# exanauts/SqpSolver.jl

Hardware: AMD Instinct MI355X
Metric: QP subproblems/sec on batched ACOPF; fp64 KKT LDL^T TFLOPS vs MFMA peak (higher is better)
Workload: dtype f64

## Files before the change

include/sqphip_test_hooks.h:

```cpp
#ifndef SQPHIP_TEST_HOOKS_H
#define SQPHIP_TEST_HOOKS_H
#include "sqphip.h"
#ifdef __cplusplus
extern "C" {
#endif

int sqphip_mf_host_solve(int64_t n, int64_t m, int64_t nnzJ, const int64_t *jrow, const int64_t *jcol,
                         int64_t nnzH, const int64_t *hrow, const int64_t *hcol, const double *gL, const double *gU,
                         int32_t condense, const double *Jval, const double *Hval, const double *Dd,
                         const double *sigp, const double *hd, const int32_t *rtype, double hsc, double dw,
                         const double *rhs, double *sol, double *dinv_by_unknown, int32_t *npos);
double sqphip_mf_host_top2_err(void);
double sqphip_mf_host_spine_err(void);
int sqphip_mf_solve_test(sqphip_ctx *ctx, int32_t inst, const double *Jval, const double *Hval, const double *Dd,
                         const double *sigp, const double *hd, const int32_t *rtype, double hsc, double dw,
                         const double *rhs, double *sol_fused, double *sol_standalone, double *dinv_by_unknown);
int sqphip_mf_batch_test(sqphip_ctx *ctx, const int32_t *active, const double *Jval, const double *Hval, const double *Dd,
                         const double *sigp, const double *hd, const int32_t *rtype, const double *hsc, const double *dw,
                         const double *dw_last, const int32_t *fac_attempt, const double *rhs, double *sol_fused,
                         double *sol_standalone, double *dinv0, double *dinv1, int32_t *decision, double *dw_out);
int sqphip_mf_values_test(sqphip_ctx *ctx, const int32_t *active, const double *Jval, const double *Hval, const double *Dd,
                          const double *sigp, const double *hd, const int32_t *rtype, const double *hsc, const double *dw,
                          const double *dw_last, const int32_t *fac_attempt, double sentinel, double *vals0, double *vals1,
                          int64_t *nnzK);
int sqphip_mf_values_blocks(int64_t n, int64_t m, int64_t nnzJ, const int64_t *jrow, const int64_t *jcol, int64_t nnzH,
                            const int64_t *hrow, const int64_t *hcol, const double *gL, const double *gU, int32_t condense,
                            const double *Jval, const double *Hval, const double *Dd, const double *sigp, const double *hd,
                            const int32_t *rtype, double hsc, double dw, int32_t *blocks, int32_t cap_blocks,
                            int32_t *n_blocks, int32_t *item_ptr, int64_t cap_dest, int64_t *n_dest, int64_t *n_items,
                            double *vals_list, double *vals_block);
int sqphip_mf_census(const sqphip_ctx *ctx, int64_t *counts, char *names, int32_t cap, int32_t *n_kernels);
int sqphip_trans_inline_groups(const sqphip_ctx *ctx, int64_t *count);
int sqphip_mf_plan_info(int64_t n, int64_t m, int64_t nnzJ, const int64_t *jrow, const int64_t *jcol, int64_t nnzH,
                        const int64_t *hrow, const int64_t *hcol, const double *gL, const double *gU, int32_t condense,
                        int32_t batch, int32_t *fronts, int32_t cap_fronts, int32_t *n_fronts, int32_t *launches,
                        int32_t cap_launches, int32_t *n_launches, int64_t *top2_lds_bytes, int32_t *spine_fronts);
int sqphip_ldlt_factor_host(int32_t device, int32_t batch, int64_t N, double *A, double *dinv,
                            int32_t *npos);
int sqphip_ldlt_solve_host(int32_t device, int32_t batch, int64_t N, const double *A,
                           double *rhs);
int sqphip_ldlt_bench(int32_t device, int32_t batch, int64_t N, int32_t reps,
                      double *sec_per_factor, double *sec_trailing, int64_t *trailing_launches);
int sqphip_ldlt_tile_masks(int32_t batch, int64_t N, const double *A, int32_t Ts, uint8_t *tmask, int32_t *pair_ptr,
                           int32_t *pair_k, int32_t cap_k, int32_t *n_k);
int sqphip_ldlt_case_test(int32_t device, int32_t batch, int64_t N, const double *A, int32_t nan_upper, const double *rhs,
                          const int32_t *phase, int32_t want, int32_t Ts, int32_t no_tile_mask, double sentinel,
                          double *factor, double *dinv, int32_t *npos, double *b, double *v, double *x_fused,
                          double *x_standalone, int64_t *counts, char *names, int32_t cap, int64_t *info);

int sqphip_ldlt_stress(int32_t device, int32_t batch, int64_t N, int32_t reps, int32_t *mismatches);
int sqphip_mfma_f64_peak(int32_t device, double *tflops);

int sqphip_seat_peek(sqphip_ctx *ctx, int32_t inst, double *p, double *lambda, double *mult_x_U, double *mult_x_L,
                     double *slack, int32_t *moi_status);

#ifdef __cplusplus
}
#endif
#endif
// ... 1 lines not shown
```

sqpsolver.jl_amd/__init__.py:

```python
from . import acopf_synth
from . import dense_synth
from . import qcqp
from . import nlp_terms
from . import _lib
from . import host
from .host import (Context, QpData, QpHip, default_options, SqpHipError, kkt_order,
                   kkt_symbolic, mf_host_solve, mf_host_top2_err, mf_host_spine_err, mf_plan_info, mf_values_blocks)
```

sqpsolver.jl_amd/_lib.py:

```python
from __future__ import annotations

import ctypes as C
import os
import subprocess
import sys

_CSRC = os.path.join(os.path.dirname(os.path.abspath(__file__)), "csrc")
SO_PATH = os.path.join(_CSRC, "libsqphip.so")
if os.environ.get("SQPHIP_SO"):
    SO_PATH = os.path.abspath(os.environ["SQPHIP_SO"])
SOURCES = ["ldlt.hip", "kernel_api.hip", "ipm.hip", "acopf.hip", "sqp.hip", "api.hip", "order.hip", "symbolic.hip",
           "mfplan.hip", "mfront.hip", "comm.hip"]
HEADERS = ["sqphip_internal.hpp", "ctx.hpp", "sparse.hpp", "dev_util.hpp", "mf_dev.hpp", "sqp_dev.hpp", "acopf_dev.hpp", "qcqp_dev.hpp", "nlp_dev.hpp", os.path.join("..", "..", "include", "sqphip.h"),
           os.path.join("..", "..", "include", "sqphip_test_hooks.h")]

_lib = None


EXTRA_FLAGS = {"mfront.hip": ["-mllvm", "-amdgpu-mfma-vgpr-form", "-mllvm", "-pragma-unroll-threshold=131072"]}
_OBJ = os.path.join(_CSRC, "build")


def build(force: bool = False, verbose: bool = False) -> str:
    from concurrent.futures import ThreadPoolExecutor
# ... 166 lines not shown
            L.sqphip_acopf_set_dclines.argtypes = [vp, C.c_int32, dp]
            L.sqphip_kkt_order.argtypes = [C.c_int64, C.c_int64, C.c_int64, lp, lp, C.c_int64, lp, lp, dp, dp, C.c_int32,
                                           ip, ip, ip]
            L.sqphip_kkt_symbolic.argtypes = [C.c_int64, C.c_int64, C.c_int64, lp, lp, C.c_int64, lp, lp, dp, dp, C.c_int32,
                                              C.c_int32, C.c_int32, C.c_double, ip, C.POINTER(SymbolicStats)]
            L.sqphip_mf_host_solve.argtypes = [C.c_int64, C.c_int64, C.c_int64, lp, lp, C.c_int64, lp, lp, dp, dp, C.c_int32,
                                               dp, dp, dp, dp, dp, ip, C.c_double, C.c_double, dp, dp, dp, ip]
            L.sqphip_mf_host_top2_err.argtypes = []
            L.sqphip_mf_host_top2_err.restype = C.c_double
            L.sqphip_mf_host_spine_err.argtypes = []
            L.sqphip_mf_host_spine_err.restype = C.c_double
            L.sqphip_mf_solve_test.argtypes = [vp, C.c_int32, dp, dp, dp, dp, dp, ip, C.c_double, C.c_double, dp, dp, dp, dp]
            L.sqphip_mf_batch_test.argtypes = [vp, ip, dp, dp, dp, dp, dp, ip, dp, dp, dp, ip, dp, dp, dp, dp, dp, ip, dp]
            L.sqphip_mf_census.argtypes = [vp, lp, C.c_char_p, C.c_int32, ip]
            if not os.environ.get("SQPHIP_SO") or hasattr(L, "sqphip_mf_values_test"):
                L.sqphip_mf_values_test.argtypes = [vp, ip, dp, dp, dp, dp, dp, ip, dp, dp, dp, ip, C.c_double, dp, dp, lp]
                L.sqphip_mf_values_blocks.argtypes = [C.c_int64, C.c_int64, C.c_int64, lp, lp, C.c_int64, lp, lp, dp, dp, C.c_int32,
                                                      dp, dp, dp, dp, dp, ip, C.c_double, C.c_double, ip, C.c_int32, ip, ip,
                                                      C.c_int64, lp, lp, dp, dp]
            if hasattr(L, "sqphip_trans_inline_groups"):
                L.sqphip_trans_inline_groups.argtypes = [vp, lp]
            L.sqphip_mf_plan_info.argtypes = [C.c_int64, C.c_int64, C.c_int64, lp, lp, C.c_int64, lp, lp, dp, dp, C.c_int32,
                                              C.c_int32, ip, C.c_int32, ip, ip, C.c_int32, ip, lp, ip]
            L.sqphip_acopf_eval.argtypes = [vp, C.c_int32, dp, C.c_double, dp, dp, dp, dp, dp, dp]
            L.sqphip_sqp_reset.argtypes = [vp]
            L.sqphip_sqp_run.argtypes = [vp, C.c_int32]
            L.sqphip_sqp_get.argtypes = [vp, C.c_int32, dp, dp, dp, dp, dp, dp, ip, ip]
            L.sqphip_sqp_status.argtypes = [vp, ip, ip, ip]
            L.sqphip_sqp_trace.argtypes = [vp, C.c_int32, dp, C.c_int32, ip]
            L.sqphip_comm_unique_id.argtypes = [vp]
            L.sqphip_comm_init.argtypes = [vp, vp, C.c_int32, C.c_int32]
            L.sqphip_gather_status.argtypes = [vp, C.c_int32, ip, ip, ip]
            L.sqphip_comm_destroy.argtypes = [vp]
            L.sqphip_get_counters.argtypes = [vp, C.POINTER(Counters)]
            L.sqphip_get_mode_counters.argtypes = [vp, C.POINTER(C.c_int64)]
            L.sqphip_sqp_qp_log.argtypes = [vp, C.c_int32, ip, C.c_int32, ip]
            L.sqphip_sqp_last_request.argtypes = [vp, C.c_int32, ip, dp, dp, dp, dp, dp, dp, dp]
            L.sqphip_sqp_stream_begin.argtypes = [vp, C.c_int32]
            L.sqphip_sqp_stream_set.argtypes = [vp, C.c_int32] + [dp] * 8
            L.sqphip_sqp_stream_run.argtypes = [vp]
            L.sqphip_sqp_stream_get.argtypes = [vp, C.c_int32, dp, dp, ip, ip]
            L.sqphip_qcqp_stream_begin.argtypes = [vp, C.c_int32, C.c_int32]
            L.sqphip_qcqp_stream_set.argtypes = [vp, C.c_int32] + [dp] * 11
            L.sqphip_sqp_stream_get_full.argtypes = [vp, C.c_int32, dp, dp, dp, dp, dp, dp, ip, ip]
            if not os.environ.get("SQPHIP_SO") or hasattr(L, "sqphip_nlp_stream_begin"):
                L.sqphip_nlp_stream_begin.argtypes = [vp, C.c_int32, C.c_int32]
                L.sqphip_nlp_stream_set.argtypes = [vp, C.c_int32] + [dp] * 8
            L.sqphip_sqp_work.argtypes = [vp, C.POINTER(C.c_int64), C.POINTER(C.c_int64), C.POINTER(C.c_int64)]
            L.sqphip_reset_counters.argtypes = [vp]
            L.sqphip_set_timing.argtypes = [vp, C.c_int32]
            L.sqphip_get_kernel_times.argtypes = [vp, dp, C.POINTER(C.c_int64), C.c_int32]
        _lib = L
    return _lib


EXPORTS = [
    "sqphip_default_options", "sqphip_create", "sqphip_destroy", "sqphip_last_error",
    "sqphip_set_bounds", "sqphip_qp_solve", "sqphip_qp_stats",
    "sqphip_qp_solve_batch", "sqphip_qp_stats_batch", "sqphip_seat_peek", "sqphip_norm_violations_batch", "sqphip_kt_residuals_batch",
    "sqphip_norm_complementarity_batch", "sqphip_compute_phi_batch", "sqphip_compute_qmodel_batch",
    "sqphip_compute_derivative_full_batch", "sqphip_qp_termination", "sqphip_sqp_qp_log_term", "sqphip_get_termination_counters", "sqphip_norm_violations",
    "sqphip_kt_residuals", "sqphip_norm_complementarity", "sqphip_compute_phi",
    "sqphip_compute_qmodel", "sqphip_compute_derivative", "sqphip_compute_derivative_full", "sqphip_compute_mu_rule_dev",
    "sqphip_acopf_armijo", "sqphip_tr_update",
    "sqphip_kkt_order", "sqphip_kkt_symbolic", "sqphip_mf_host_solve", "sqphip_mf_host_top2_err", "sqphip_mf_host_spine_err", "sqphip_mf_solve_test", "sqphip_mf_batch_test", "sqphip_mf_values_test", "sqphip_mf_values_blocks", "sqphip_mf_census", "sqphip_trans_inline_groups", "sqphip_mf_plan_info", "sqphip_acopf_attach", "sqphip_acopf_attach_acr", "sqphip_acopf_attach_acwr", "sqphip_acopf_set_shunts", "sqphip_acopf_set_dclines", "sqphip_acopf_set_instance", "sqphip_dense_attach", "sqphip_dense_set_instance", "sqphip_qcqp_attach", "sqphip_qcqp_set_instance", "sqphip_nlp_attach", "sqphip_nlp_attach_affine", "sqphip_nlp_set_instance", "sqphip_acopf_eval", "sqphip_sqp_reset",
    "sqphip_sqp_run", "sqphip_sqp_get", "sqphip_sqp_status", "sqphip_sqp_trace",
    "sqphip_comm_available", "sqphip_comm_unique_id", "sqphip_comm_init", "sqphip_gather_status", "sqphip_comm_destroy",
    "sqphip_get_counters", "sqphip_get_mode_counters", "sqphip_sqp_work", "sqphip_sqp_stream_begin", "sqphip_sqp_stream_set", "sqphip_sqp_stream_run", "sqphip_sqp_stream_get", "sqphip_sqp_stream_assign", "sqphip_sqp_stream_append", "sqphip_sqp_stream_release", "sqphip_sqp_stream_run_some", "sqphip_qcqp_stream_begin", "sqphip_qcqp_stream_set", "sqphip_nlp_stream_begin", "sqphip_nlp_stream_set", "sqphip_sqp_stream_get_full", "sqphip_sqp_last_request", "sqphip_sqp_qp_log", "sqphip_reset_counters", "sqphip_set_timing", "sqphip_get_kernel_times", "sqphip_ldlt_factor_host",
    "sqphip_ldlt_solve_host", "sqphip_ldlt_bench", "sqphip_ldlt_stress", "sqphip_ldlt_tile_masks", "sqphip_ldlt_case_test", "sqphip_mfma_f64_peak", "sqphip_armijo_alpha", "sqphip_compute_mu_rule",
]
```

sqpsolver.jl_amd/csrc/api.hip:

```cpp
#include "ctx.hpp"
#include "qcqp_dev.hpp"
#include "nlp_dev.hpp"
#include <algorithm>
#include <array>
#include <chrono>
#include <cmath>
#include <cstring>
#include <tuple>
#include <unordered_map>

using namespace sqphip;

Ctx::~Ctx()
{
    lanes.clear();
    tm.flush();
    comm_release(*this);
    plan.destroy_lookahead();
    for (void *p : allocs) hipFree(p);
    if (h_counters) hipHostFree(h_counters);
    if (stg_h) hipHostFree(stg_h);
    if (side) { hipStreamDestroy(side); for (auto &e : evS) if (e) hipEventDestroy(e); for (auto &e : evC) if (e) hipEventDestroy(e); }
    if (stream && owns_stream) hipStreamDestroy(stream);
}
// ... 1858 lines not shown
        for (auto &s : S) { nqp += s.n_qp; nip += s.tot_ipm; nf += s.tot_fac; nsol += s.tot_sol; }
        c->n_qp = nqp; c->n_ipm_iter = nip; c->n_factor = nf;
        const double N = (double)C.d.Nf;
        c->kkt_order = C.d.Nf;
        c->lead_tiles = C.d.Ts;
        c->trailing_flops_per_factor = ldlt_trailing_flops(C.plan);
        c->ldlt_flops = (double)nf * N * N * N / 3.0;
        c->ldlt_seconds = C.tm.factor_seconds + lane_factor; c->trailing_seconds = C.tm.trailing_seconds + lane_trailing;
        c->solve_seconds = C.tm.solve_seconds + lane_solve; c->total_seconds = C.total_seconds;
        c->trailing_launches = C.tm.trailing_launches;
        c->n_sweeps = C.n_sweeps + lane_sweeps; c->n_solve = nsol; c->n_groups = C.lanes.empty() ? 1 : (int64_t)C.lanes.size();
        c->sparse = C.d.sparse; c->nnz_k = 0; c->nnz_l = 0; c->n_supernodes = 0; c->n_levels = 0; c->max_front = 0;
        c->factor_flops = 0; c->front_doubles = 0; c->cb_doubles = 0; c->factor_launches = 0; c->solve_launches = 0;
        c->nnz_l_top = 0; c->nnz_k_top = 0; c->cols_top = 0;
        if (C.d.sparse) {
            const SparseSym &Y = C.mfp().S;
            c->nnz_k = C.mfp().nnzK; c->nnz_l = Y.nnzL; c->n_supernodes = Y.ns; c->n_levels = Y.nlevels;
            c->max_front = Y.max_front; c->factor_flops = Y.flops; c->front_doubles = C.mfp().stride;
            long cb = 0;
            for (int q = 0; q < Y.ns; ++q) cb += (long)(Y.sn_nr[q] + 1) * Y.sn_nr[q] - (long)Y.sn_nr[q] * (Y.sn_nr[q] - 1) / 2;
            c->cb_doubles = cb;
            long lt = 0, kt = 0, nct = 0;
            for (int q = 0; q < Y.ns; ++q)
                if (Y.sn_level[q] >= C.mfp().narrow_level) {
                    const long nc = Y.sn_nc[q], nr = Y.sn_nr[q];
                    lt += nc * (nc - 1) / 2 + nc * nr; kt += C.mfp().asm_ptr[q + 1] - C.mfp().asm_ptr[q]; nct += nc;
                }
            c->nnz_l_top = lt; c->nnz_k_top = kt; c->cols_top = nct;
            c->factor_launches = (int64_t)(C.d.mf.sp_n > 0 ? C.mfp().fac_below + 1 : (int)C.mfp().fac.size());
            c->solve_launches = (int64_t)(C.mfp().fwd.size() + C.mfp().bwd.size() + (C.mfp().top.count > 0 ? 1 : 0));
            c->ldlt_flops = (double)nf * Y.flops;
        }
        return SQPHIP_OK;
    });
}

extern "C" int sqphip_get_mode_counters(sqphip_ctx *h, int64_t *out)
{
    if (!h || !out) return SQPHIP_EINVAL;
    return guarded(h, [&](Ctx &C) -> int {
        for (int k = 0; k < 12; ++k) out[k] = 0;
        if (!C.d.sst) return SQPHIP_OK;
        std::vector<SqpState> S((size_t)C.d.B);
        SQPHIP_HIP_OK(hipMemcpyAsync(S.data(), C.d.sst, sizeof(SqpState) * C.d.B, hipMemcpyDeviceToHost, C.stream));
        SQPHIP_HIP_OK(hipStreamSynchronize(C.stream));
        for (auto &s : S)
            for (int k = 0; k < 4; ++k) { out[3 * k] += s.md_qp[k]; out[3 * k + 1] += s.md_ipm[k]; out[3 * k + 2] += s.md_fac[k]; }
// ... 463 lines not shown
```

sqpsolver.jl_amd/csrc/mfplan.hip:

```cpp
#include "sparse.hpp"
#include "../../include/sqphip.h"
#include "../../include/sqphip_test_hooks.h"
#include <algorithm>
#include <cmath>
#include <cstdio>
#include <cstdlib>
#include <tuple>

namespace sqphip {

MfPlan mf_build_plan(int n, int m, const std::vector<int> &kpos, int mk, const std::vector<int> &hcolptr,
                     const std::vector<int> &hrowval, const std::vector<int> &jrowptr, const std::vector<int> &jrcol,
                     const std::vector<int> &jrslot, const SymOptions &opt)
{
    MfPlan P;
    std::vector<std::vector<int>> adj, before;
    kkt_graph(n, m, kpos, mk, hcolptr, hrowval, jrowptr, jrcol, adj, before);
    P.S = sparse_symbolic(n + mk, adj, before, opt);
    const SparseSym &S = P.S;
    P.off.resize(S.ns);
    for (int s = 0; s < S.ns; ++s) {
        const long fs = S.sn_nc[s] + S.sn_nr[s];
        P.off[s] = P.stride;
        P.stride += ((fs + 1) * fs + 1) / 2 * 2;
// ... 141 lines not shown
        }
        for (int s = 0; s < S.ns; ++s) P.ev_ptr[s + 1] += P.ev_ptr[s];
    }
    auto tiles = [&](int s) { return (S.sn_nc[s] + S.sn_nr[s] + 1 + 15) / 16; };
    auto cls = [&](int s) { const int T = tiles(s); return T <= 2 ? 1 : (T <= 6 ? T - 1 : (T <= 8 ? 7 : (T <= 13 ? 8 : 9))); };
    for (int l = 0; l < S.nlevels; ++l) {
        int cnt = 0, tmax = 0;
        for (int q = S.level_ptr[l]; q < S.level_ptr[l + 1]; ++q) { ++cnt; tmax = std::max(tmax, tiles(S.level_sn[q])); }
        const int merge_t = getenv("SQPHIP_MF_MERGE_T") ? atoi(getenv("SQPHIP_MF_MERGE_T")) : opt.merge_tiles;
        const bool merge = ((cnt <= 8 && tmax <= 8) || tmax <= merge_t) && !getenv("SQPHIP_MF_NO_LEVEL_MERGE");
        for (int c = 0; c < 10; ++c) {
            MfLaunch L{(int)P.sched.size(), 0, 0, 0, c, 0};
            L.level = l;
            for (int q = S.level_ptr[l]; q < S.level_ptr[l + 1]; ++q) {
                const int s = S.level_sn[q];
                if (merge ? c != tmax - 1 : cls(s) != c) continue;
                P.sched.push_back(s);
                L.count++;
                L.tiles = std::max(L.tiles, tiles(s));
            }
            if (!L.count) continue;
            if (!merge && c == 1) L.tiles = 2;
            if (!merge && c == 7) L.tiles = 8;
            P.fac.push_back(L);
        }
    }
    auto build_solve_launches = [&]() {
    P.sol_items.clear(); P.fwd.clear(); P.bwd.clear(); P.top = MfLaunch{0, 0, 256, 0, 0, 0};
    int top_maxfs = 64, top_lcap = 0;
    for (int l = 0; l < S.nlevels; ++l) {
        const bool top = l >= P.top_level;
        MfLaunch L{(int)P.sol_items.size() / 4, 0, 256, 0, 0, 0};
        int maxfs = 64, lcap = 0;
        std::vector<int> small;
        for (int q = S.level_ptr[l]; q < S.level_ptr[l + 1]; ++q) {
            const int s = S.level_sn[q], fs = S.sn_nc[s] + S.sn_nr[s];
            if (!big_solve) maxfs = std::max(maxfs, fs);
            if (fs > 64 && big_solve) {
                for (int t : {s, -2, -2, -2}) P.sol_items.push_back(t);
                maxfs = std::max(maxfs, fs);
                const int nc = S.sn_nc[s];
                if (nc <= 80) lcap = std::max(lcap, nc * nc);
            } else small.push_back(s);
        }
        for (size_t q = 0; q < small.size(); q += 4)
            for (size_t t = q; t < q + 4; ++t) P.sol_items.push_back(t < small.size() ? small[t] : -1);
// ... 135 lines not shown
                for (int t = 0; t < nr; ++t) P.sp_rel.push_back(S.rel[S.sn_rowptr[s] + t]);
                P.sp_rel.push_back(pfs);
                P.spine_stage = std::max(P.spine_stage, (nr + 1) * nr);
            }
            P.sp_fr.push_back(F);
        }
        if (ok && !P.sp_fr.empty()) {
            const int R = 16 * P.spine_T;
            P.spine_stage = (P.spine_stage + 1) / 2 * 2;
            P.spine_lds_bytes = 8L * ((long)R * R + 256 + 40 + R + 64 * 8 + P.spine_stage + 136);
            if (P.spine_lds_bytes > 160 * 1024 - 1024) ok = false;
        }
        if (!ok || P.sp_fr.empty()) { P.sp_fr.clear(); P.sp_ent.clear(); P.sp_src.clear(); P.sp_rel.clear(); P.spine_lds_bytes = 0; P.spine_level = S.nlevels; P.fac_below = (int)P.fac.size(); }
        if (getenv("SQPHIP_SYM_DUMP"))
            for (const MfSpineFront &F : P.sp_fr) {
                int hist[5] = {0, 0, 0, 0, 0};
                for (int t = F.ea_begin; t < F.ea_end; ++t) hist[std::min(4, P.sp_ent[t].src_end - P.sp_ent[t].src_begin)]++;
                fprintf(stderr, "  spine front %d: %d x %d, T %d, %d structural entries, %d receiving entries from the arena (1 / 2 / 3 / 4+ sources: %d / %d / %d / %d), handoff %d\n",
                        F.s, F.nc, F.nr, F.T, F.asm_end - F.asm_begin, F.ea_end - F.ea_begin, hist[1], hist[2], hist[3], hist[4], F.handoff);
            }
        if (getenv("SQPHIP_SYM_DUMP"))
            fprintf(stderr, "spine (factorisation): %d fronts from level %d, tallest %d tiles, %zu arena gather entries, LDS %ld bytes\n",
                    (int)P.sp_fr.size(), P.spine_level, P.spine_T, P.sp_ent.size(), P.spine_lds_bytes);
    }
    return P;
}

static inline double item_value(const MfItem &it, const MfValues &V)
{
    const double reg_p = 1e-8, reg_d = 1e-8;
    switch (it.type) {
    case MF_ITEM_H: return V.hsc * V.hv[it.a];
    case MF_ITEM_JKEPT: return V.rtype[it.row] != 0 ? V.jv[it.a] : 0.0;
    case MF_ITEM_PAIR: return V.rtype[it.row] != 0 ? V.jv[it.a] * V.jv[it.b] / (V.Dd[it.row] + reg_d) : 0.0;
    case MF_ITEM_VDIAG: return V.hd[it.a] + V.sigp[it.a] + V.dw + reg_p;
    default: return V.rtype[it.row] != 0 ? -(V.Dd[it.row] + reg_d) : -1.0;
    }
}

static double g_top2_err = -1.0;
static double g_spine_err = -1.0;

void mf_host_factor_solve(const MfPlan &P, const MfValues &V, const double *rhs, double *sol, double *dinv)
{
    const SparseSym &S = P.S;
    std::vector<double> F(P.stride, 0.0), x(S.nu), v(S.nu);
// ... 262 lines not shown
        (cap_launches > 0 && !launches))
        return SQPHIP_EINVAL;
    using namespace sqphip;
    const SymOptions so = mf_sym_options(batch);
    std::vector<double> jv, hv;
    const MfPlan P = host_plan(n, m, nnzJ, jrow, jcol, nnzH, hrow, hcol, gL, gU, condense, so, nullptr, nullptr, jv, hv);
    const SparseSym &S = P.S;
    std::vector<int> level(S.ns, 0);
    for (int l = 0; l < S.nlevels; ++l)
        for (int q = S.level_ptr[l]; q < S.level_ptr[l + 1]; ++q) level[S.level_sn[q]] = l;
    for (int f = 0; f < S.ns && f < cap_fronts; ++f) { fronts[3 * f] = S.sn_nc[f]; fronts[3 * f + 1] = S.sn_nr[f]; fronts[3 * f + 2] = level[f]; }
    for (int k = 0; k < (int)P.fac.size() && k < cap_launches; ++k) {
        const MfLaunch &L = P.fac[k];
        int tmin = 1 << 30;
        for (int q = L.begin; q < L.begin + L.count; ++q) tmin = std::min(tmin, (S.sn_nc[P.sched[q]] + S.sn_nr[P.sched[q]] + 1 + 15) / 16);
        launches[4 * k] = L.level; launches[4 * k + 1] = L.tiles; launches[4 * k + 2] = L.count; launches[4 * k + 3] = tmin;
    }
    if (n_fronts) *n_fronts = S.ns;
    if (n_launches) *n_launches = (int32_t)P.fac.size();
    if (top2_lds_bytes) *top2_lds_bytes = P.top2_lds_bytes;
    if (spine_fronts) *spine_fronts = (int32_t)P.sp_fr.size();
    return SQPHIP_OK;
}
```

sqpsolver.jl_amd/csrc/mfront.hip:

```cpp
#include "ctx.hpp"
#include "dev_util.hpp"
#include "mf_dev.hpp"
#include <cstdlib>
#include <mutex>

namespace sqphip {

#ifdef SQPHIP_MF_TRACE
__device__ long long g_mf_trace[1 << 16][8];
#define MF_TR(i) if (inst == 0 && threadIdx.x == 0 && s < (1 << 16)) g_mf_trace[s][i] = (long long)wall_clock64();
__device__ long long g_mf_trace2[1 << 12][16];
#define MF_TRW(i) if (W == 0 && trs >= 0 && trs < (1 << 12) && lane == 0) g_mf_trace2[trs][i] = (long long)clock64();
__device__ long long g_mf_trace3[1 << 12][16];
#define MF_TRS(i) if (inst == 0 && tid == 0 && s < (1 << 12)) g_mf_trace3[s][i] = (long long)clock64();
#define MF_TR2S(a, b) if (inst == 0 && lane == 0 && j < 64 && wave < 2) g_mf_trace3[(do_fwd ? 64 : 0) + j][wave == 0 ? (a) : (b)] = (long long)clock64();
#define MF_TR2W(c) if (trj >= 0 && lane == 0) g_mf_trace3[trj][c] = (long long)clock64();
#define MF_TRSP(c) if (inst == 0 && cand == 0 && tid == 0 && k < 64) g_mf_trace3[128 + k][c] = (long long)wall_clock64();
#else
#define MF_TR(i)
#define MF_TRW(i)
#define MF_TRS(i)
#define MF_TR2S(a, b)
#define MF_TR2W(c)
#define MF_TRSP(c)
// ... 1753 lines not shown
    big(reinterpret_cast<const void *>(k_mf_front<6, 4, true>)); big(reinterpret_cast<const void *>(k_mf_front<7, 4, true>));
    big(reinterpret_cast<const void *>(k_mf_front<8, 4, true>)); big(reinterpret_cast<const void *>(k_mf_front<6, 8, true>));
    big(reinterpret_cast<const void *>(k_mf_front<7, 8, true>)); big(reinterpret_cast<const void *>(k_mf_front<8, 8, true>));
    big(reinterpret_cast<const void *>(k_mf_fwd2<true>)); big(reinterpret_cast<const void *>(k_mf_bwd2<true>));
    big(reinterpret_cast<const void *>(k_mf_fwd2<false>)); big(reinterpret_cast<const void *>(k_mf_bwd2<false>));
    big(reinterpret_cast<const void *>(k_mf_solve_top2));
    big(reinterpret_cast<const void *>(k_mf_spine));
    (void)hipGetLastError();
    C.mf_big_lds = ok;
}

void mf_values(Ctx &C, int want)
{
    const DV &d = C.d;
    hipStream_t s = C.stream;
    const int nb = d.mf.fronts1 && d.spec_mode != 0 ? 2 * d.B : d.B;
    const bool serial = d.mf.nvblk == 0 || (getenv("SQPHIP_MF_VALUES_SERIAL") && atoi(getenv("SQPHIP_MF_VALUES_SERIAL")) != 0);
    C.tm.open(s); C.mf_census[MFK_VALUES]++;
    if (serial) hipLaunchKernelGGL(k_mf_values_serial, dim3((d.mf.nnzK + 255) / 256, nb), dim3(256), 0, s, d, want);
    else hipLaunchKernelGGL(k_mf_values, dim3(d.mf.nvblk, nb), dim3(MF_VBLK_ITEMS), 0, s, d, want);
    C.tm.close(KC_VALUES, s);
}

void mf_factor(Ctx &C, int want, bool with_rhs, bool values_done)
{
    const DV &d = C.d;
    hipStream_t s = C.stream;
    static const bool v1 = getenv("SQPHIP_MF_V1") != nullptr;
    const int wr = (int)with_rhs;
    const int nb = d.mf.fronts1 && d.spec_mode != 0 ? 2 * d.B : d.B;
    if (!v1 && !values_done) mf_values(C, want);
    const bool stat = !(getenv("SQPHIP_MF_STATIC") && atoi(getenv("SQPHIP_MF_STATIC")) == 0);
    const bool packed = !(getenv("SQPHIP_MF_F2_PACKED") && atoi(getenv("SQPHIP_MF_F2_PACKED")) == 0);
    const bool spine = !v1 && d.mf.sp_n > 0 && C.mf_big_lds;
    int li = 0, cls_open = -1;
    for (const MfLaunch &L : C.mfp().fac) {
        if (spine && li++ >= C.mfp().fac_below) break;
        const int cls = L.level >= C.mfp().narrow_level ? KC_FRONTS_TOP : KC_FRONTS_LOW;
        if (cls != cls_open) { if (cls_open >= 0) C.tm.close(cls_open, s); C.tm.open(s); cls_open = cls; }
        const dim3 grid(L.count, nb);
        const int T = L.tiles;
        if (v1 || T > 13) { C.mf_census[MFK_FACTOR_R1]++; hipLaunchKernelGGL((k_mf_factor<256, true>), grid, dim3(256), 0, s, d, L.begin, want, wr); continue; }
#define MF_GENERIC(NW, MAXT, IMG) do { constexpr int kid_ = mf_factor2_kid(NW, MAXT, IMG); static_assert(kid_ >= 0, "census: no counter"); C.mf_census[kid_]++; \
        if (IMG && packed) hipLaunchKernelGGL((k_mf_factor2<NW, MAXT, IMG, IMG>), grid, dim3(64 * NW), 8 * mf_factor2_lds_doubles(T, IMG, true), s, d, L.begin, want, wr, T); \
        else hipLaunchKernelGGL((k_mf_factor2<NW, MAXT, IMG, false>), grid, dim3(64 * NW), 8 * mf_factor2_lds_doubles(T, IMG, false), s, d, L.begin, want, wr, T); } while (0)
#define MF_STATIC(TT, NW, IMG) do { constexpr int kid_ = mf_front_kid(TT, NW, IMG); static_assert(kid_ >= 0, "census: no counter"); C.mf_census[kid_]++; hipLaunchKernelGGL((k_mf_front<TT, NW, IMG>), grid, dim3(64 * NW), 8 * (size_t)mf_front_lds_doubles(TT, NW, IMG), s, d, L.begin, want, wr); } while (0)
        const int stat_min = getenv("SQPHIP_MF_STATIC_MIN") ? atoi(getenv("SQPHIP_MF_STATIC_MIN")) : (L.count <= 8 && L.level >= C.mfp().narrow_level ? 1 : 4);
        const bool nw8 = !(getenv("SQPHIP_MF_NW8") && atoi(getenv("SQPHIP_MF_NW8")) == 0);
        const int nw4 = L.count <= 8 ? (getenv("SQPHIP_MF_NW4") ? atoi(getenv("SQPHIP_MF_NW4")) : 3) : 0;
        const bool big_img = C.mf_big_lds && !(getenv("SQPHIP_MF_BIG_LDSIMG") && atoi(getenv("SQPHIP_MF_BIG_LDSIMG")) == 0);
        static const int stat_max = getenv("SQPHIP_MF_STATIC_MAX") ? atoi(getenv("SQPHIP_MF_STATIC_MAX")) : 12;
        if (!stat || T > stat_max || T > 12 || T < stat_min) {
            if (T <= 2) MF_GENERIC(1, 3, true);
            else if (T <= 4) MF_GENERIC(2, 5, true);
            else if (T <= 5) MF_GENERIC(4, 4, true);
            else if (T <= 8) MF_GENERIC(4, 9, false);
            else MF_GENERIC(8, 12, false);
            continue;
        }
        switch (T) {
        case 1: MF_STATIC(1, 1, true); break;
        case 2: MF_STATIC(2, 1, true); break;
        case 3: MF_STATIC(3, 1, true); break;
        case 4: if (nw4 & 1) MF_STATIC(4, 4, true); else MF_STATIC(4, 2, true); break;
        case 5: if (nw4 & 2) MF_STATIC(5, 4, true); else MF_STATIC(5, 2, true); break;
        case 6: if (big_img && L.count <= 8) { if (nw8) MF_STATIC(6, 8, true); else MF_STATIC(6, 4, true); } else MF_STATIC(6, 4, false); break;
        case 7: if (big_img && L.count <= 8) { if (nw8) MF_STATIC(7, 8, true); else MF_STATIC(7, 4, true); } else MF_STATIC(7, 4, false); break;
        case 8: if (big_img && L.count <= 8) { if (nw8) MF_STATIC(8, 8, true); else MF_STATIC(8, 4, true); } else MF_STATIC(8, 4, false); break;
        case 9: MF_STATIC(9, 8, false); break;
        case 10: MF_STATIC(10, 8, false); break;
        case 11: MF_STATIC(11, 8, false); break;
        default: MF_STATIC(12, 8, false); break;
        }
#undef MF_GENERIC
#undef MF_STATIC
    }
    if (cls_open >= 0) C.tm.close(cls_open, s);
    if (spine) { C.tm.open(s); C.mf_census[MFK_SPINE]++; hipLaunchKernelGGL(k_mf_spine, dim3(1, nb), dim3(MF_SP_NT), (size_t)C.mfp().spine_lds_bytes, s, d, want, wr); C.tm.close(KC_FRONTS_TOP, s); }
    C.mf_factor_launches += spine ? (long)C.mfp().fac_below + 1 : (long)C.mfp().fac.size();
}

bool mf_solve_tests_inertia(const Ctx &C)
{
    static const bool off = getenv("SQPHIP_MF_INERTIA_KERNEL") != nullptr;
    return !off && C.d.sparse && C.d.mf.top_n > 0 && !mf_generic_solves() && !(C.d.B >= (getenv("SQPHIP_MF_INST_SOLVE_MIN") ? atoi(getenv("SQPHIP_MF_INST_SOLVE_MIN")) : (1 << 30)));
}

void mf_solve(Ctx &C, int want, bool skip_fwd, bool inertia, int also)
{
    const DV &d = C.d;
    hipStream_t s = C.stream;
// ... 49 lines not shown
```

sqpsolver.jl_amd/csrc/sparse.hpp:

```cpp
#pragma once
#include <cstdint>
#include <cstdlib>
#include <vector>

namespace sqphip {

struct SparseSym {
    int nu = 0;
    std::vector<int> pos, inv;
    int ns = 0;
    std::vector<int> sn_first, sn_nc, sn_nr, sn_rowptr, sn_rows, sn_parent, sn_level;
    std::vector<int> col2sn;
    std::vector<int> rel;
    std::vector<int> child_ptr, child;
    std::vector<long> front_off;
    long front_total = 0;
    int nlevels = 0;
    std::vector<int> level_ptr, level_sn;
    long nnzL = 0;
    long nnzL_exact = 0;
    double flops = 0;
    double flops_exact = 0;
    int max_front = 0, max_nc = 0;
};
// ... 19 lines not shown
    return so;
}

SparseSym sparse_symbolic(int nu, const std::vector<std::vector<int>> &adj, const std::vector<std::vector<int>> &before,
                          const SymOptions &opt);

void kkt_graph(int n, int m, const std::vector<int> &kpos, int mk, const std::vector<int> &hcolptr,
               const std::vector<int> &hrowval, const std::vector<int> &jrowptr, const std::vector<int> &jrcol,
               std::vector<std::vector<int>> &adj, std::vector<std::vector<int>> &before);

enum { MF_ITEM_H = 0,
       MF_ITEM_JKEPT = 1,
       MF_ITEM_PAIR = 2,
       MF_ITEM_VDIAG = 3,
       MF_ITEM_RDIAG = 4 };
struct MfItem { int type, row, a, b; };

constexpr int MF_VBLK_ITEMS = 256;
struct MfValBlock { int dest0, item0, ndest, nitems; };

struct MfFrontDesc { int nc, nr, first, rowptr, off, asm_begin, asm_end, ea_begin, ea_end, ev_begin, ev_end, pad; };
struct MfGather { int where, src_begin, src_end, src0; };

struct MfLaunch { int begin, count, threads, lds_bytes, cls, tiles; int wimg = -1, lds2 = 0, hasbig = 1; int level = 0; };

struct MfTopFront { int s, nc, nr, first, off, ll, xloc, uoff, gptr, gsrc0, nsrc, rloc, lbuf, pad0, pad1, pad2; };

struct MfSpineFront { int s, nc, nr, first, off, T, asm_begin, asm_end, ea_begin, ea_end, handoff, rel, pad0, pad1, pad2, pad3; };

struct MfPlan {
    SparseSym S;
    std::vector<long> off;
    long stride = 0;
    std::vector<int> asm_ptr, dest_loc, item_ptr;
    std::vector<MfItem> items;
    std::vector<MfItem> vitems;
    std::vector<MfValBlock> vblk;
    std::vector<int> dest_rc;
    std::vector<int> ea_ptr, ea_rc, ea_src_ptr, ea_src;
    std::vector<int> ev_ptr, ev_idx, ev_src_ptr, ev_src;
    std::vector<int> sol_items;
    std::vector<MfFrontDesc> desc;
    std::vector<MfGather> ea_ent, ev_ent;
    std::vector<int> sched;
    std::vector<MfLaunch> fac, fwd, bwd;
    MfLaunch top{0, 0, 256, 0, 0, 0};
    int top_level = 0;
    std::vector<MfTopFront> top_fr;
    std::vector<int> top_gptr, top_gsrc, top_rows, top_ext;
    int top_xtotal = 0, top_utotal = 0, top_buf0 = 0, top_buf1 = 0;
    long top2_lds_bytes = 0;
    long nnzK = 0;
    int spine_level = 0, spine_T = 0;
    int narrow_level = 0;
    std::vector<MfSpineFront> sp_fr;
    std::vector<MfGather> sp_ent;
    std::vector<int> sp_src, sp_rel;
    long spine_lds_bytes = 0;
    int spine_stage = 0;
    int fac_below = 0;
};

MfPlan mf_build_plan(int n, int m, const std::vector<int> &kpos, int mk, const std::vector<int> &hcolptr,
                     const std::vector<int> &hrowval, const std::vector<int> &jrowptr, const std::vector<int> &jrcol,
                     const std::vector<int> &jrslot, const SymOptions &opt);

struct MfValues { const double *hv, *jv, *Dd, *sigp, *hd; const int *rtype; double hsc, dw; };
void mf_host_factor_solve(const MfPlan &P, const MfValues &V, const double *rhs, double *sol, double *dinv);
// ... 3 lines not shown
```

sqpsolver.jl_amd/host.py:

```python
from __future__ import annotations

import ctypes as C
import dataclasses
import math
import numpy as np

from . import _lib

MODE_QP, MODE_FR, MODE_SOC, MODE_LP, MODE_L1QP, MODE_INFEAS = range(6)
LOCALLY_SOLVED, LOCALLY_INFEASIBLE, ITERATION_LIMIT, NUMERICAL_ERROR = 4, 5, 11, 20
_OK = (1, 7, 10, 4)
_INFEAS = (2, 5)

_dp = C.POINTER(C.c_double)


def _d(a):
    return None if a is None else a.ctypes.data_as(_dp)


def _f(a):
    return None if a is None else np.ascontiguousarray(a, dtype=np.float64)


# ... 57 lines not shown
        raise SqpHipError(f"sqphip_mf_host_solve failed ({rc})")
    return sol, dinv, npos.value


def mf_host_top2_err() -> float:
    return float(_lib.lib().sqphip_mf_host_top2_err())


def mf_host_spine_err() -> float:
    return float(_lib.lib().sqphip_mf_host_spine_err())


def mf_plan_info(n, m, jrow, jcol, hrow, hcol, gL, gU, condense=1, batch=1):
    L = _lib.lib()
    jr, jc, hr, hc = (np.ascontiguousarray(a, dtype=np.int64) for a in (jrow, jcol, hrow, hcol))
    nf, nl, top, sp = C.c_int32(), C.c_int32(), C.c_int64(), C.c_int32()
    args = (n, m, len(jr), _l(jr), _l(jc), len(hr), _l(hr), _l(hc), _d(_f(gL)), _d(_f(gU)), int(condense), int(batch))
    if L.sqphip_mf_plan_info(*args, None, 0, C.byref(nf), None, 0, C.byref(nl), C.byref(top), C.byref(sp)) != 0:
        raise SqpHipError("sqphip_mf_plan_info failed")
    fr = np.zeros((nf.value, 3), dtype=np.int32); la = np.zeros((nl.value, 4), dtype=np.int32)
    if L.sqphip_mf_plan_info(*args, _i(fr), nf.value, C.byref(nf), _i(la), nl.value, C.byref(nl), C.byref(top), C.byref(sp)) != 0:
        raise SqpHipError("sqphip_mf_plan_info failed")
    return fr, la, top.value, sp.value


def mf_values_blocks(n, m, jrow, jcol, hrow, hcol, gL, gU, condense=1, values=None):
    L = _lib.lib()
    jr, jc, hr, hc = (np.ascontiguousarray(a, dtype=np.int64) for a in (jrow, jcol, hrow, hcol))
    nb, nd, ni = C.c_int32(), C.c_int64(), C.c_int64()
    head = (n, m, len(jr), _l(jr), _l(jc), len(hr), _l(hr), _l(hc), _d(_f(gL)), _d(_f(gU)), int(condense))
    none = (None, None, None, None, None, None, 0.0, 0.0)
    if L.sqphip_mf_values_blocks(*head, *none, None, 0, C.byref(nb), None, 0, C.byref(nd), C.byref(ni), None, None) != 0:
        raise SqpHipError("sqphip_mf_values_blocks failed")
    blocks = np.zeros((nb.value, 4), dtype=np.int32); ptr = np.zeros(nd.value + 1, dtype=np.int32)
    out = {"blocks": blocks, "item_ptr": ptr, "n_items": ni.value, "vals_list": None, "vals_block": None}
    vals = none; vl = vb = None
    if values is not None:
        jval, hval, Dd, sigp, hd, rtype, hsc, dw = values
        rt = np.ascontiguousarray(rtype, dtype=np.int32)
        vals = (_d(_f(jval)), _d(_f(hval)), _d(_f(Dd)), _d(_f(sigp)), _d(_f(hd)), _i(rt), float(hsc), float(dw))
        vl = np.zeros(nd.value); vb = np.zeros(nd.value)
    if L.sqphip_mf_values_blocks(*head, *vals, _i(blocks) if nb.value else None, nb.value, C.byref(nb), _i(ptr), nd.value,
                                 C.byref(nd), C.byref(ni), _d(vl) if vl is not None else None,
                                 _d(vb) if vb is not None else None) != 0:
        raise SqpHipError("sqphip_mf_values_blocks failed")
    if values is not None:
# ... 593 lines not shown
```

Baseline: 10160.

## Defer multifrontal factor fronts into later compatible launches to cut launch count

Adds a planning pass that moves every front of a factor launch into later launches with the same kernel selection, provided each is still below its parent's level. A launch whose fronts can all be moved is removed, so fewer level-by-level factor kernels run and the remaining ones get wider grids. The pass is on by default, can be switched with an environment variable, and runs only when there is no spine. It records each launch's small/narrow properties so kernel choice stays the same after the merge. It also adds a test hook that reports the front-to-launch mapping, and the cost accounting now uses the launch's level instead of the front's own level.

```diff
diff --git a/include/sqphip_test_hooks.h b/include/sqphip_test_hooks.h
--- a/include/sqphip_test_hooks.h
+++ b/include/sqphip_test_hooks.h
@@ -35,6 +35,9 @@
                         const int64_t *hrow, const int64_t *hcol, const double *gL, const double *gU, int32_t condense,
                         int32_t batch, int32_t *fronts, int32_t cap_fronts, int32_t *n_fronts, int32_t *launches,
                         int32_t cap_launches, int32_t *n_launches, int64_t *top2_lds_bytes, int32_t *spine_fronts);
+int sqphip_mf_front_launches(int64_t n, int64_t m, int64_t nnzJ, const int64_t *jrow, const int64_t *jcol, int64_t nnzH,
+                             const int64_t *hrow, const int64_t *hcol, const double *gL, const double *gU, int32_t condense,
+                             int32_t batch, int32_t *fronts, int32_t cap_fronts, int32_t *n_fronts);
 int sqphip_ldlt_factor_host(int32_t device, int32_t batch, int64_t N, double *A, double *dinv,
                             int32_t *npos);
 int sqphip_ldlt_solve_host(int32_t device, int32_t batch, int64_t N, const double *A,
diff --git a/sqpsolver.jl_amd/__init__.py b/sqpsolver.jl_amd/__init__.py
--- a/sqpsolver.jl_amd/__init__.py
+++ b/sqpsolver.jl_amd/__init__.py
@@ -5,4 +5,4 @@
 from . import _lib
 from . import host
 from .host import (Context, QpData, QpHip, default_options, SqpHipError, kkt_order,
-                   kkt_symbolic, mf_host_solve, mf_host_top2_err, mf_host_spine_err, mf_plan_info, mf_values_blocks)
+                   kkt_symbolic, mf_host_solve, mf_host_top2_err, mf_host_spine_err, mf_plan_info, mf_front_launches, mf_values_blocks)
diff --git a/sqpsolver.jl_amd/_lib.py b/sqpsolver.jl_amd/_lib.py
--- a/sqpsolver.jl_amd/_lib.py
+++ b/sqpsolver.jl_amd/_lib.py
@@ -212,6 +212,9 @@
                 L.sqphip_trans_inline_groups.argtypes = [vp, lp]
             L.sqphip_mf_plan_info.argtypes = [C.c_int64, C.c_int64, C.c_int64, lp, lp, C.c_int64, lp, lp, dp, dp, C.c_int32,
                                               C.c_int32, ip, C.c_int32, ip, ip, C.c_int32, ip, lp, ip]
+            if not os.environ.get("SQPHIP_SO") or hasattr(L, "sqphip_mf_front_launches"):
+                L.sqphip_mf_front_launches.argtypes = [C.c_int64, C.c_int64, C.c_int64, lp, lp, C.c_int64, lp, lp, dp, dp, C.c_int32,
+                                                       C.c_int32, ip, C.c_int32, ip]
             L.sqphip_acopf_eval.argtypes = [vp, C.c_int32, dp, C.c_double, dp, dp, dp, dp, dp, dp]
             L.sqphip_sqp_reset.argtypes = [vp]
             L.sqphip_sqp_run.argtypes = [vp, C.c_int32]
@@ -253,7 +256,7 @@
     "sqphip_kt_residuals", "sqphip_norm_complementarity", "sqphip_compute_phi",
     "sqphip_compute_qmodel", "sqphip_compute_derivative", "sqphip_compute_derivative_full", "sqphip_compute_mu_rule_dev",
     "sqphip_acopf_armijo", "sqphip_tr_update",
-    "sqphip_kkt_order", "sqphip_kkt_symbolic", "sqphip_mf_host_solve", "sqphip_mf_host_top2_err", "sqphip_mf_host_spine_err", "sqphip_mf_solve_test", "sqphip_mf_batch_test", "sqphip_mf_values_test", "sqphip_mf_values_blocks", "sqphip_mf_census", "sqphip_trans_inline_groups", "sqphip_mf_plan_info", "sqphip_acopf_attach", "sqphip_acopf_attach_acr", "sqphip_acopf_attach_acwr", "sqphip_acopf_set_shunts", "sqphip_acopf_set_dclines", "sqphip_acopf_set_instance", "sqphip_dense_attach", "sqphip_dense_set_instance", "sqphip_qcqp_attach", "sqphip_qcqp_set_instance", "sqphip_nlp_attach", "sqphip_nlp_attach_affine", "sqphip_nlp_set_instance", "sqphip_acopf_eval", "sqphip_sqp_reset",
+    "sqphip_kkt_order", "sqphip_kkt_symbolic", "sqphip_mf_host_solve", "sqphip_mf_host_top2_err", "sqphip_mf_host_spine_err", "sqphip_mf_solve_test", "sqphip_mf_batch_test", "sqphip_mf_values_test", "sqphip_mf_values_blocks", "sqphip_mf_census", "sqphip_trans_inline_groups", "sqphip_mf_plan_info", "sqphip_mf_front_launches", "sqphip_acopf_attach", "sqphip_acopf_attach_acr", "sqphip_acopf_attach_acwr", "sqphip_acopf_set_shunts", "sqphip_acopf_set_dclines", "sqphip_acopf_set_instance", "sqphip_dense_attach", "sqphip_dense_set_instance", "sqphip_qcqp_attach", "sqphip_qcqp_set_instance", "sqphip_nlp_attach", "sqphip_nlp_attach_affine", "sqphip_nlp_set_instance", "sqphip_acopf_eval", "sqphip_sqp_reset",
     "sqphip_sqp_run", "sqphip_sqp_get", "sqphip_sqp_status", "sqphip_sqp_trace",
     "sqphip_comm_available", "sqphip_comm_unique_id", "sqphip_comm_init", "sqphip_gather_status", "sqphip_comm_destroy",
     "sqphip_get_counters", "sqphip_get_mode_counters", "sqphip_sqp_work", "sqphip_sqp_stream_begin", "sqphip_sqp_stream_set", "sqphip_sqp_stream_run", "sqphip_sqp_stream_get", "sqphip_sqp_stream_assign", "sqphip_sqp_stream_append", "sqphip_sqp_stream_release", "sqphip_sqp_stream_run_some", "sqphip_qcqp_stream_begin", "sqphip_qcqp_stream_set", "sqphip_nlp_stream_begin", "sqphip_nlp_stream_set", "sqphip_sqp_stream_get_full", "sqphip_sqp_last_request", "sqphip_sqp_qp_log", "sqphip_reset_counters", "sqphip_set_timing", "sqphip_get_kernel_times", "sqphip_ldlt_factor_host",
diff --git a/sqpsolver.jl_amd/csrc/api.hip b/sqpsolver.jl_amd/csrc/api.hip
--- a/sqpsolver.jl_amd/csrc/api.hip
+++ b/sqpsolver.jl_amd/csrc/api.hip
@@ -1904,7 +1904,7 @@
             c->cb_doubles = cb;
             long lt = 0, kt = 0, nct = 0;
             for (int q = 0; q < Y.ns; ++q)
-                if (Y.sn_level[q] >= C.mfp().narrow_level) {
+                if (C.mfp().fac[C.mfp().launch_of[q]].level >= C.mfp().narrow_level) {
                     const long nc = Y.sn_nc[q], nr = Y.sn_nr[q];
                     lt += nc * (nc - 1) / 2 + nc * nr; kt += C.mfp().asm_ptr[q + 1] - C.mfp().asm_ptr[q]; nct += nc;
                 }
diff --git a/sqpsolver.jl_amd/csrc/mfplan.hip b/sqpsolver.jl_amd/csrc/mfplan.hip
--- a/sqpsolver.jl_amd/csrc/mfplan.hip
+++ b/sqpsolver.jl_amd/csrc/mfplan.hip
@@ -187,6 +187,7 @@
             if (!L.count) continue;
             if (!merge && c == 1) L.tiles = 2;
             if (!merge && c == 7) L.tiles = 8;
+            L.small = L.count <= 8;
             P.fac.push_back(L);
         }
     }
@@ -368,6 +369,66 @@
         if (getenv("SQPHIP_SYM_DUMP"))
             fprintf(stderr, "spine (factorisation): %d fronts from level %d, tallest %d tiles, %zu arena gather entries, LDS %ld bytes\n",
                     (int)P.sp_fr.size(), P.spine_level, P.spine_T, P.sp_ent.size(), P.spine_lds_bytes);
+    }
+    {
+        const int defer = getenv("SQPHIP_MF_DEFER") ? atoi(getenv("SQPHIP_MF_DEFER")) : 1;
+        const int nl = (int)P.fac.size();
+        std::vector<std::vector<int>> mem(nl);
+        P.launch_of0.assign(S.ns, -1);
+        for (int k = 0; k < nl; ++k)
+            for (int q = P.fac[k].begin; q < P.fac[k].begin + P.fac[k].count; ++q) { mem[k].push_back(P.sched[q]); P.launch_of0[P.sched[q]] = k; }
+        std::vector<char> alive(nl, 1);
+        if (defer != 0 && P.sp_fr.empty()) {
+            std::vector<int> width(nl, 0);
+            for (int k = 0; k < nl; ++k) {
+                int fs = -1;
+                for (int s : mem[k]) {
+                    const int h = S.sn_nc[s] + S.sn_nr[s];
+                    if (h > fs || (h == fs && S.sn_nc[s] > width[k])) { fs = h; width[k] = S.sn_nc[s]; }
+                }
+            }
+            std::vector<int> dest;
+            for (int a = 0; a < nl; ++a) {
+                const MfLaunch &A = P.fac[a];
+                dest.clear();
+                for (int s : mem[a]) {
+                    const int p = S.sn_parent[s], bound = p >= 0 ? S.sn_level[p] : S.nlevels;
+                    int best = -1;
+                    for (int b = a + 1; b < nl && P.fac[b].level < bound; ++b) {
+                        const MfLaunch &B = P.fac[b];
+                        if (!alive[b] || B.level <= A.level || !mf_same_selection(A, B, P.narrow_level)) continue;
+                        if (best < 0 || defer != 2 || width[b] >= width[best]) best = b;
+                    }
+                    if (best < 0) break;
+                    dest.push_back(best);
+                }
+                if (dest.size() != mem[a].size()) continue;
+                for (size_t t = 0; t < dest.size(); ++t) mem[dest[t]].push_back(mem[a][t]);
+                mem[a].clear(); alive[a] = 0;
+            }
+            std::vector<MfLaunch> fac;
+            P.sched.clear();
+            for (int k = 0; k < nl; ++k) {
+                if (!alive[k]) continue;
+                MfLaunch L = P.fac[k];
+                L.begin = (int)P.sched.size(); L.count = (int)mem[k].size();
+                P.sched.insert(P.sched.end(), mem[k].begin(), mem[k].end());
+                fac.push_back(L);
+            }
+            P.fac.swap(fac);
+            P.fac_below = (int)P.fac.size();
+        }
+        P.launch_of.assign(S.ns, -1);
+        for (int k = 0; k < (int)P.fac.size(); ++k)
+            for (int q = P.fac[k].begin; q < P.fac[k].begin + P.fac[k].count; ++q) P.launch_of[P.sched[q]] = k;
+        if (getenv("SQPHIP_SYM_DUMP")) {
+            for (int s = 0; s < S.ns; ++s)
+                if (alive[P.launch_of0[s]] == 0)
+                    fprintf(stderr, "  deferred: front %d (%d x %d, level %d, parent's level %d) from launch %d to launch %d (level %d)\n", s, S.sn_nc[s],
+                            S.sn_nr[s], S.sn_level[s], S.sn_parent[s] >= 0 ? S.sn_level[S.sn_parent[s]] : -1, P.launch_of0[s], P.launch_of[s],
+                            P.fac[P.launch_of[s]].level);
+            fprintf(stderr, "factor launches: %d (%d before deferral)\n", (int)P.fac.size(), nl);
+        }
     }
     return P;
 }
@@ -676,3 +737,18 @@
     if (spine_fronts) *spine_fronts = (int32_t)P.sp_fr.size();
     return SQPHIP_OK;
 }
+
+extern "C" int sqphip_mf_front_launches(int64_t n, int64_t m, int64_t nnzJ, const int64_t *jrow, const int64_t *jcol, int64_t nnzH,
+                                        const int64_t *hrow, const int64_t *hcol, const double *gL, const double *gU,
+                                        int32_t condense, int32_t batch, int32_t *fronts, int32_t cap_fronts, int32_t *n_fronts)
+{
+    if (n <= 0 || m < 0 || batch <= 0 || cap_fronts < 0 || (cap_fronts > 0 && !fronts)) return SQPHIP_EINVAL;
+    using namespace sqphip;
+    const SymOptions so = mf_sym_options(batch);
+    std::vector<double> jv, hv;
+    const MfPlan P = host_plan(n, m, nnzJ, jrow, jcol, nnzH, hrow, hcol, gL, gU, condense, so, nullptr, nullptr, jv, hv);
+    const SparseSym &S = P.S;
+    for (int f = 0; f < S.ns && f < cap_fronts; ++f) { fronts[3 * f] = P.launch_of[f]; fronts[3 * f + 1] = P.launch_of0[f]; fronts[3 * f + 2] = S.sn_parent[f]; }
+    if (n_fronts) *n_fronts = S.ns;
+    return SQPHIP_OK;
+}
diff --git a/sqpsolver.jl_amd/csrc/mfront.hip b/sqpsolver.jl_amd/csrc/mfront.hip
--- a/sqpsolver.jl_amd/csrc/mfront.hip
+++ b/sqpsolver.jl_amd/csrc/mfront.hip
@@ -1799,6 +1799,13 @@
     C.tm.close(KC_VALUES, s);
 }
 
+static inline bool mf_launch_narrow(const MfLaunch &L, int narrow_level) { return L.level >= narrow_level; }
+bool mf_same_selection(const MfLaunch &a, const MfLaunch &b, int narrow_level)
+{
+    return a.tiles == b.tiles && a.small == b.small &&
+           (a.tiles >= 4 || mf_launch_narrow(a, narrow_level) == mf_launch_narrow(b, narrow_level));
+}
+
 void mf_factor(Ctx &C, int want, bool with_rhs, bool values_done)
 {
     const DV &d = C.d;
@@ -1813,7 +1820,7 @@
     int li = 0, cls_open = -1;
     for (const MfLaunch &L : C.mfp().fac) {
         if (spine && li++ >= C.mfp().fac_below) break;
-        const int cls = L.level >= C.mfp().narrow_level ? KC_FRONTS_TOP : KC_FRONTS_LOW;
+        const int cls = mf_launch_narrow(L, C.mfp().narrow_level) ? KC_FRONTS_TOP : KC_FRONTS_LOW;
         if (cls != cls_open) { if (cls_open >= 0) C.tm.close(cls_open, s); C.tm.open(s); cls_open = cls; }
         const dim3 grid(L.count, nb);
         const int T = L.tiles;
@@ -1822,9 +1829,9 @@
         if (IMG && packed) hipLaunchKernelGGL((k_mf_factor2<NW, MAXT, IMG, IMG>), grid, dim3(64 * NW), 8 * mf_factor2_lds_doubles(T, IMG, true), s, d, L.begin, want, wr, T); \
         else hipLaunchKernelGGL((k_mf_factor2<NW, MAXT, IMG, false>), grid, dim3(64 * NW), 8 * mf_factor2_lds_doubles(T, IMG, false), s, d, L.begin, want, wr, T); } while (0)
 #define MF_STATIC(TT, NW, IMG) do { constexpr int kid_ = mf_front_kid(TT, NW, IMG); static_assert(kid_ >= 0, "census: no counter"); C.mf_census[kid_]++; hipLaunchKernelGGL((k_mf_front<TT, NW, IMG>), grid, dim3(64 * NW), 8 * (size_t)mf_front_lds_doubles(TT, NW, IMG), s, d, L.begin, want, wr); } while (0)
-        const int stat_min = getenv("SQPHIP_MF_STATIC_MIN") ? atoi(getenv("SQPHIP_MF_STATIC_MIN")) : (L.count <= 8 && L.level >= C.mfp().narrow_level ? 1 : 4);
+        const int stat_min = getenv("SQPHIP_MF_STATIC_MIN") ? atoi(getenv("SQPHIP_MF_STATIC_MIN")) : (L.small && mf_launch_narrow(L, C.mfp().narrow_level) ? 1 : 4);
         const bool nw8 = !(getenv("SQPHIP_MF_NW8") && atoi(getenv("SQPHIP_MF_NW8")) == 0);
-        const int nw4 = L.count <= 8 ? (getenv("SQPHIP_MF_NW4") ? atoi(getenv("SQPHIP_MF_NW4")) : 3) : 0;
+        const int nw4 = L.small ? (getenv("SQPHIP_MF_NW4") ? atoi(getenv("SQPHIP_MF_NW4")) : 3) : 0;
         const bool big_img = C.mf_big_lds && !(getenv("SQPHIP_MF_BIG_LDSIMG") && atoi(getenv("SQPHIP_MF_BIG_LDSIMG")) == 0);
         static const int stat_max = getenv("SQPHIP_MF_STATIC_MAX") ? atoi(getenv("SQPHIP_MF_STATIC_MAX")) : 12;
         if (!stat || T > stat_max || T > 12 || T < stat_min) {
@@ -1841,9 +1848,9 @@
         case 3: MF_STATIC(3, 1, true); break;
         case 4: if (nw4 & 1) MF_STATIC(4, 4, true); else MF_STATIC(4, 2, true); break;
         case 5: if (nw4 & 2) MF_STATIC(5, 4, true); else MF_STATIC(5, 2, true); break;
-        case 6: if (big_img && L.count <= 8) { if (nw8) MF_STATIC(6, 8, true); else MF_STATIC(6, 4, true); } else MF_STATIC(6, 4, false); break;
-        case 7: if (big_img && L.count <= 8) { if (nw8) MF_STATIC(7, 8, true); else MF_STATIC(7, 4, true); } else MF_STATIC(7, 4, false); break;
-        case 8: if (big_img && L.count <= 8) { if (nw8) MF_STATIC(8, 8, true); else MF_STATIC(8, 4, true); } else MF_STATIC(8, 4, false); break;
+        case 6: if (big_img && L.small) { if (nw8) MF_STATIC(6, 8, true); else MF_STATIC(6, 4, true); } else MF_STATIC(6, 4, false); break;
+        case 7: if (big_img && L.small) { if (nw8) MF_STATIC(7, 8, true); else MF_STATIC(7, 4, true); } else MF_STATIC(7, 4, false); break;
+        case 8: if (big_img && L.small) { if (nw8) MF_STATIC(8, 8, true); else MF_STATIC(8, 4, true); } else MF_STATIC(8, 4, false); break;
         case 9: MF_STATIC(9, 8, false); break;
         case 10: MF_STATIC(10, 8, false); break;
         case 11: MF_STATIC(11, 8, false); break;
diff --git a/sqpsolver.jl_amd/csrc/sparse.hpp b/sqpsolver.jl_amd/csrc/sparse.hpp
--- a/sqpsolver.jl_amd/csrc/sparse.hpp
+++ b/sqpsolver.jl_amd/csrc/sparse.hpp
@@ -65,7 +65,8 @@
 struct MfFrontDesc { int nc, nr, first, rowptr, off, asm_begin, asm_end, ea_begin, ea_end, ev_begin, ev_end, pad; };
 struct MfGather { int where, src_begin, src_end, src0; };
 
-struct MfLaunch { int begin, count, threads, lds_bytes, cls, tiles; int wimg = -1, lds2 = 0, hasbig = 1; int level = 0; };
+struct MfLaunch { int begin, count, threads, lds_bytes, cls, tiles; int wimg = -1, lds2 = 0, hasbig = 1; int level = 0; int small = 0; };
+bool mf_same_selection(const MfLaunch &a, const MfLaunch &b, int narrow_level);
 
 struct MfTopFront { int s, nc, nr, first, off, ll, xloc, uoff, gptr, gsrc0, nsrc, rloc, lbuf, pad0, pad1, pad2; };
 
@@ -87,6 +88,7 @@
     std::vector<MfGather> ea_ent, ev_ent;
     std::vector<int> sched;
     std::vector<MfLaunch> fac, fwd, bwd;
+    std::vector<int> launch_of, launch_of0;
     MfLaunch top{0, 0, 256, 0, 0, 0};
     int top_level = 0;
     std::vector<MfTopFront> top_fr;
diff --git a/sqpsolver.jl_amd/host.py b/sqpsolver.jl_amd/host.py
--- a/sqpsolver.jl_amd/host.py
+++ b/sqpsolver.jl_amd/host.py
@@ -103,6 +103,19 @@
     if L.sqphip_mf_plan_info(*args, _i(fr), nf.value, C.byref(nf), _i(la), nl.value, C.byref(nl), C.byref(top), C.byref(sp)) != 0:
         raise SqpHipError("sqphip_mf_plan_info failed")
     return fr, la, top.value, sp.value
+
+
+def mf_front_launches(n, m, jrow, jcol, hrow, hcol, gL, gU, condense=1, batch=1):
+    L = _lib.lib()
+    jr, jc, hr, hc = (np.ascontiguousarray(a, dtype=np.int64) for a in (jrow, jcol, hrow, hcol))
+    nf = C.c_int32()
+    args = (n, m, len(jr), _l(jr), _l(jc), len(hr), _l(hr), _l(hc), _d(_f(gL)), _d(_f(gU)), int(condense), int(batch))
+    if L.sqphip_mf_front_launches(*args, None, 0, C.byref(nf)) != 0:
+        raise SqpHipError("sqphip_mf_front_launches failed")
+    fr = np.zeros((nf.value, 3), dtype=np.int32)
+    if L.sqphip_mf_front_launches(*args, _i(fr), nf.value, C.byref(nf)) != 0:
+        raise SqpHipError("sqphip_mf_front_launches failed")
+    return fr
 
 
 def mf_values_blocks(n, m, jrow, jcol, hrow, hcol, gL, gU, condense=1, values=None):
```

Result: faster. 10360, median of 6 (+1.9%).
